# neuzxy/Distributed-TF-Serving

Measured on AMD Instinct MI355X. Metric: CTR scores/sec (whole node), higher is better.
Workload: dtype bf16; 1 GPU; model=deepfm (1Mx64 emb, 43 fields, MLP 1024-512-256), global_batch=16384, request_rows=512, parallelism=candidate-dp1 (one GPU, no fan-out), encoding=raw, aux_lane_cus=0

## Files before the change

### csrc/bindings_native.cpp

```cpp
#include <torch/extension.h>

#include <pybind11/stl.h>

#include <algorithm>
#include <cstring>

#include "runtime/batcher.h"
#include "runtime/arena.h"
#include "runtime/thread_pool.h"
#include "runtime/trace.h"
#include "wire/tensor_codec.h"
#include "live_bindings.h"
#include "runtime/narrow.h"
#include "net/hpack.h"
#include "runtime/numa.h"
#include "net/h2_client.h"

namespace py = pybind11;
using namespace dtfs;

namespace {

wire::DstType dst_type_of(const torch::Tensor& t) {
  switch (t.scalar_type()) {
    case torch::kInt32: return wire::DstType::I32;
    case torch::kInt64: return wire::DstType::I64;
    case torch::kFloat32: return wire::DstType::F32;
    case torch::kBFloat16: return wire::DstType::BF16;
    default: throw py::value_error("decode destination must be int32, int64, float32 or bfloat16");
  }
}

int wire_dtype_of(const torch::Tensor& t) {
  switch (t.scalar_type()) {
    case torch::kFloat32: return wire::DT_FLOAT;
    case torch::kFloat64: return wire::DT_DOUBLE;
    case torch::kInt32: return wire::DT_INT32;
    case torch::kInt64: return wire::DT_INT64;
    case torch::kBFloat16: return wire::DT_BFLOAT16;
    case torch::kFloat16: return wire::DT_HALF;
    default: throw py::value_error("unsupported tensor dtype for encoding");
  }
}

struct ParsedRequest {
  py::bytes holder;
  std::string storage;
  wire::PredictRequestView view;

  const wire::TensorView& get(const std::string& key) const {
    const wire::TensorView* t = view.find(key);
    if (!t) throw py::key_error("input '" + key + "' not found in PredictRequest");
    return *t;
  }
};

std::shared_ptr<ParsedRequest> parse_request(py::bytes data) {
// ... 192 lines not shown
      errs[k] = "input '" + b.ids_key + "': " + err;
      return;
    }
    if (wbase && b.wts_t[i]) {
      wire::DecodeOpts ow;
      ow.dst = wt;
      ow.cols = b.fields;
      ow.ld = wld;
      const bool ok = whole ? wire::decode_into(*b.wts_t[i], wbase + size_t(row * wld) * wes, n, ow, &err)
                            : wire::decode_into(sub(*b.wts_t[i], e0, e1), wbase + size_t(row * wld) * wes, n, ow, &err);
      if (!ok) errs[k] = "input '" + b.wts_key + "': " + err;
    }
  });
  for (size_t k = 0; k < items.size(); ++k)
    if (!errs[k].empty() && b.errors[items[k].req].empty()) b.errors[items[k].req] = errs[k];
}

using runtime::ArenaBatch;
using runtime::kArenaMaxRequests;
using runtime::kArenaPayloadOff;

void check_arena(const torch::Tensor& arena) {
  if (arena.device().type() != torch::kCPU || !arena.is_contiguous() || arena.scalar_type() != torch::kUInt8)
    throw py::value_error("arena must be a contiguous CPU uint8 tensor");
}

std::vector<std::pair<int64_t, int64_t>> arena_place(torch::Tensor arena, const std::vector<py::bytes>& reqs,
                                                     int64_t start) {
  check_arena(arena);
  std::vector<std::pair<const char*, size_t>> src(reqs.size());
  for (size_t i = 0; i < reqs.size(); ++i) {
    char* p;
    Py_ssize_t len;
    if (PyBytes_AsStringAndSize(reqs[i].ptr(), &p, &len) != 0) throw py::error_already_set();
    src[i] = {p, size_t(len)};
  }
  py::gil_scoped_release nogil;
  try {
    return runtime::arena_place(arena.data_ptr<uint8_t>(), arena.numel(), src, start);
  } catch (const std::invalid_argument& e) {
    py::gil_scoped_acquire g;
    throw py::value_error(e.what());
  }
}

ArenaBatch arena_build(torch::Tensor arena, const std::vector<std::pair<int64_t, int64_t>>& spans,
                       const std::string& ids_key, const std::string& wts_key, int64_t fields, int64_t max_rows,
                       int64_t varint_chunks, int64_t n_ranked) {
  check_arena(arena);
  py::gil_scoped_release nogil;
  try {
    return runtime::arena_build(arena.data_ptr<uint8_t>(), arena.numel(), spans, ids_key, wts_key, fields, max_rows,
                                varint_chunks, n_ranked);
  } catch (const std::invalid_argument& e) {
    py::gil_scoped_acquire g;
    throw py::value_error(e.what());
  }
}

void arena_unpack_cpu(torch::Tensor arena, torch::Tensor packed, int64_t fields) {
  check_arena(arena);
  if (packed.scalar_type() != torch::kInt64 || packed.dim() != 2 || !packed.is_contiguous())
    throw py::value_error("packed must be a contiguous int64 [B, W] tensor");
  if (packed.size(1) * 8 < 12 * fields) throw py::value_error("packed rows too narrow for the field count");
  const uint8_t* base = arena.data_ptr<uint8_t>();
  uint8_t* dst = reinterpret_cast<uint8_t*>(packed.data_ptr<int64_t>());
  const int64_t W = packed.size(1), B = packed.size(0);
  py::gil_scoped_release nogil;
  runtime::arena_unpack_cpu(base, dst, B, W, fields);
}

std::vector<py::bytes> encode_batch_responses(const std::string& name, const std::string& sig, py::object version,
                                              const std::string& key, torch::Tensor scores,
                                              const std::vector<int64_t>& rows, const std::vector<int64_t>& offsets,
                                              bool raw) {
  if (scores.device().type() != torch::kCPU || scores.scalar_type() != torch::kFloat32 || !scores.is_contiguous())
    throw py::value_error("scores must be a contiguous CPU fp32 tensor");
  if (rows.size() != offsets.size()) throw py::value_error("rows/offsets length mismatch");
  wire::ModelSpecOut spec;
  spec.name = name;
  spec.signature_name = sig;
  if (!version.is_none()) {
    spec.has_version = true;
    spec.version = version.cast<int64_t>();
  }
  const float* s = scores.data_ptr<float>();
  const int64_t ns = scores.numel();
  std::vector<std::string> outs(rows.size());
  {
    py::gil_scoped_release nogil;
    for (size_t i = 0; i < rows.size(); ++i) {
      if (offsets[i] < 0 || rows[i] < 0 || offsets[i] + rows[i] > ns) continue;
      wire::TensorOut t;
      t.key = key;
      t.dtype = wire::DT_FLOAT;
      t.shape = {rows[i]};
      t.data = s + offsets[i];
      t.n = rows[i];
      t.raw = raw;
      outs[i] = wire::encode_predict_response(spec, {t});
    }
  }
  std::vector<py::bytes> res;
  res.reserve(outs.size());
  for (auto& o : outs) res.emplace_back(o);
  return res;
// ... 268 lines not shown
      .def_property_readonly("output_filter", [](const ParsedRequest& r) { return r.view.output_filter; })
      .def("input_names", [](const ParsedRequest& r) {
        std::vector<std::string> k;
        for (const auto& kv : r.view.inputs) k.push_back(kv.first);
        return k;
      })
      .def("has_input", [](const ParsedRequest& r, const std::string& k) { return r.view.find(k) != nullptr; })
      .def("shape", [](const ParsedRequest& r, const std::string& k) { return r.get(k).shape; })
      .def("dtype", [](const ParsedRequest& r, const std::string& k) { return r.get(k).dtype; })
      .def("num_elements", [](const ParsedRequest& r, const std::string& k) { return r.get(k).num_elements(); })
      .def("num_values", [](const ParsedRequest& r, const std::string& k) {
        const auto& t = r.get(k);
        return t.content.n ? t.num_elements() : t.num_values;
      })
      .def("is_raw", [](const ParsedRequest& r, const std::string& k) { return r.get(k).content.n > 0; })
      .def("decode_into", &decode_into, py::arg("key"), py::arg("dst"), py::arg("offset") = 0,
           py::arg("id_modulo") = 0,
           "Decode input `key` (TF fill semantics) into dst[offset: offset+numel], narrowing dtypes.");

  m.def("parse_predict_request", &parse_request, py::arg("data"));

  py::class_<ParsedBatch, std::shared_ptr<ParsedBatch>>(m, "ParsedBatch")
      .def_readonly("rows", &ParsedBatch::rows)
      .def_readonly("offsets", &ParsedBatch::offsets)
      .def_readonly("errors", &ParsedBatch::errors)
      .def_readonly("total_rows", &ParsedBatch::total_rows)
      .def_readonly("fields", &ParsedBatch::fields)
      .def("__len__", [](const ParsedBatch& b) { return b.views.size(); })
      .def("model_name", [](const ParsedBatch& b, size_t i) { return b.views.at(i).model_name; })
      .def("signature_name", [](const ParsedBatch& b, size_t i) { return b.views.at(i).signature_name; })
      .def("version", [](const ParsedBatch& b, size_t i) -> py::object {
        const auto& v = b.views.at(i);
        return v.has_version ? py::object(py::int_(v.version)) : py::object(py::none());
      })
      .def("output_filter", [](const ParsedBatch& b, size_t i) { return b.views.at(i).output_filter; })
      .def("decode", &decode_batch_range, py::arg("ids_dst"), py::arg("wts_dst"), py::arg("begin") = 0,
           py::arg("end") = int64_t(1) << 62, py::arg("base_row") = 0, py::arg("id_modulo") = 0);

  py::class_<ArenaBatch>(m, "ArenaBatch")
      .def_readonly("rows", &ArenaBatch::rows)
      .def_readonly("offsets", &ArenaBatch::offsets)
      .def_readonly("errors", &ArenaBatch::errors)
      .def_readonly("total_rows", &ArenaBatch::total_rows)
      .def_readonly("used_bytes", &ArenaBatch::used_bytes)
      .def_readonly("n_valid", &ArenaBatch::n_valid)
      .def_readonly("n_decoded", &ArenaBatch::n_decoded)
      .def_readonly("n_gpu_varint", &ArenaBatch::n_gpu_varint);
  m.attr("ARENA_PAYLOAD_OFF") = kArenaPayloadOff;
  m.attr("ARENA_MAX_REQUESTS") = kArenaMaxRequests;
  m.def("arena_place", &arena_place, py::arg("arena"), py::arg("requests"), py::arg("start") = 0);
  m.def("arena_build", &arena_build, py::arg("arena"), py::arg("spans"), py::arg("ids_key") = "feat_ids",
        py::arg("wts_key") = "feat_wts", py::arg("fields") = 43, py::arg("max_rows") = int64_t(1) << 40,
        py::arg("varint_chunks") = 0, py::arg("n_ranked") = 0);
  m.def("arena_varint_capacity", &runtime::arena_varint_capacity, py::arg("max_rows"), py::arg("fields"),
        py::arg("max_requests") = runtime::kArenaMaxRequests);
  m.def("arena_unpack_cpu", &arena_unpack_cpu, py::arg("arena"), py::arg("packed"), py::arg("fields"));

  m.def("parse_batch", &parse_batch, py::arg("requests"), py::arg("ids_key") = "feat_ids",
        py::arg("wts_key") = "feat_wts", py::arg("fields") = 43,
        "Parse many serialized PredictRequests (GIL released); see ParsedBatch.decode.");
  m.def("encode_batch_responses", &encode_batch_responses, py::arg("model_name"), py::arg("signature_name"),
        py::arg("version"), py::arg("key"), py::arg("scores"), py::arg("rows"), py::arg("offsets"),
        py::arg("raw") = false);

  m.def(
      "encode_predict_response",
      [](const std::string& name, const std::string& sig, py::object version,
         const std::vector<std::pair<std::string, torch::Tensor>>& outputs, bool raw) {
        std::vector<torch::Tensor> keep;
        auto outs = tensors_out(outputs, raw, &keep);
        auto spec = spec_of(name, sig, version);
        std::string s;
        {
          py::gil_scoped_release nogil;
          s = wire::encode_predict_response(spec, outs);
        }
        return py::bytes(s);
      },
      py::arg("model_name"), py::arg("signature_name"), py::arg("version"), py::arg("outputs"),
      py::arg("raw") = false);

  m.def(
      "encode_predict_request",
      [](const std::string& name, const std::string& sig, py::object version,
         const std::vector<std::pair<std::string, torch::Tensor>>& inputs, bool raw,
         const std::vector<std::string>& output_filter) {
        std::vector<torch::Tensor> keep;
        auto ins = tensors_out(inputs, raw, &keep);
        auto spec = spec_of(name, sig, version);
        std::string s;
        {
          py::gil_scoped_release nogil;
          s = wire::encode_predict_request(spec, ins, output_filter);
        }
        return py::bytes(s);
      },
      py::arg("model_name"), py::arg("signature_name"), py::arg("version"), py::arg("inputs"),
      py::arg("raw") = false, py::arg("output_filter") = std::vector<std::string>{});

  m.def("f32_to_bf16_bits", [](float f) { return wire::f32_to_bf16(f); });

  py::class_<runtime::BatchItem>(m, "BatchItem")
      .def_readonly("ticket", &runtime::BatchItem::ticket)
      .def_readonly("rows", &runtime::BatchItem::rows)
      .def_readonly("enqueue_us", &runtime::BatchItem::enqueue_us)
      .def_readonly("deadline_us", &runtime::BatchItem::deadline_us);
// ... 86 lines not shown
```

### csrc/kernels/common.h

```cpp
#pragma once

#include <hip/hip_runtime.h>
#include <stdint.h>

namespace dtfs {
namespace kern {

typedef __bf16 bf16;
typedef __bf16 bf16x8 __attribute__((ext_vector_type(8)));
typedef __bf16 bf16x4 __attribute__((ext_vector_type(4)));
typedef float f32x4 __attribute__((ext_vector_type(4)));
typedef float f32x16 __attribute__((ext_vector_type(16)));
typedef int i32x4 __attribute__((ext_vector_type(4)));

constexpr int kWave = 64;

__device__ __forceinline__ float bf2f(bf16 x) { return float(x); }
__device__ __forceinline__ bf16 f2bf(float x) { return (bf16)x; }

__device__ __forceinline__ float wave_sum(float v) {
#pragma unroll
  for (int o = 32; o > 0; o >>= 1) v += __shfl_xor(v, o, 64);
  return v;
}
// ... 35 lines not shown
__device__ __forceinline__ uint32_t load_u32_unaligned(const uint8_t* p) {
  const uintptr_t a = reinterpret_cast<uintptr_t>(p);
  const uint32_t* w = reinterpret_cast<const uint32_t*>(a & ~uintptr_t(3));
  const int sh = int(a & 3);
  const uint32_t w0 = w[0];
  const uint32_t w1 = sh ? w[1] : 0u;
  return __builtin_amdgcn_alignbyte(w1, w0, sh);
}

constexpr int kArenaAllWeights = 1 << 30;
__device__ __forceinline__ int arena_narrow_wcols(const uint8_t* arena) {
  const int w = *reinterpret_cast<const int32_t*>(arena + 36);
  return w > 0 ? w : kArenaAllWeights;
}

__device__ __forceinline__ int arena_narrow_idb(const uint8_t* arena) {
  return *reinterpret_cast<const int32_t*>(arena + 40) == 3 ? 3 : 4;
}

constexpr uint32_t kWtsOffMask = 0x3fffffffu;
constexpr int kWtsF32 = 0, kWtsBf16 = 1, kWtsOnes = 2;

struct ArenaRow {
  const uint8_t* ids;
  const uint8_t* wts;
  bool narrow;
  int wcols;
  int idb;
  int wkind = kWtsF32;
};

__device__ __forceinline__ int64_t arena_narrow_id(const ArenaRow& ar, int f) {
  if (ar.idb == 3) return int64_t(load_u32_unaligned(ar.ids + 3 * f) & 0xffffffu);
  return int64_t(reinterpret_cast<const int32_t*>(ar.ids)[f]);
}

__device__ __forceinline__ float arena_narrow_w(const ArenaRow& ar, int f) {
  if (f >= ar.wcols) return 0.f;
  if (ar.wkind == kWtsOnes) return 1.f;
  if (ar.wkind == kWtsBf16) return __uint_as_float(uint32_t(reinterpret_cast<const uint16_t*>(ar.wts)[f]) << 16);
  return reinterpret_cast<const float*>(ar.wts)[f];
}

__device__ __forceinline__ ArenaRow arena_row_at(const uint8_t* payload, int2 o, int wcols, int idb) {
  ArenaRow r{payload + (o.x & 0x7fffffff), payload + (uint32_t(o.y) & kWtsOffMask), o.x < 0, kArenaAllWeights, 4};
  if (r.narrow) {
    r.wcols = wcols;
    r.idb = idb;
    r.wkind = int(uint32_t(o.y) >> 30);
  }
  return r;
}

__device__ __forceinline__ ArenaRow arena_row(const uint8_t* arena, int64_t payload_off, int64_t r) {
  const int64_t total = *reinterpret_cast<const int64_t*>(arena + 8);
  ArenaRow out{nullptr, nullptr, false, kArenaAllWeights, 4};
  if (r < total) {
    const uint8_t* payload = arena + payload_off;
    const int64_t rt = *reinterpret_cast<const int64_t*>(arena + 16);
    const int2 o = reinterpret_cast<const int2*>(payload + rt)[r];
    out = arena_row_at(payload, o, arena_narrow_wcols(arena), arena_narrow_idb(arena));
  }
  return out;
}

__device__ __forceinline__ void arena_feature(const ArenaRow& ar, int f, int64_t& id, float& w) {
  if (ar.narrow) {
    id = arena_narrow_id(ar, f);
    w = arena_narrow_w(ar, f);
  } else {
    id = int64_t(load_u64_unaligned(ar.ids + 8 * f));
    w = __uint_as_float(load_u32_unaligned(ar.wts + 4 * f));
  }
}

__device__ __forceinline__ int xcd_remap(int orig, int nwg) {
  constexpr int NX = 8;
  if (nwg <= NX) return orig;
  const int q = nwg / NX, r = nwg % NX;
  const int xcd = orig % NX, slot = orig / NX;
  const int base = xcd < r ? xcd * (q + 1) : r * (q + 1) + (xcd - r) * q;
  return base + slot;
}

}
}
```

### csrc/kernels/gather_mlp.hip

```cpp
#include <utility>

#include "asm_io.h"
#include "common.h"
#include "launchers.h"

namespace dtfs {
namespace kern {

typedef __bf16 bf16x2 __attribute__((ext_vector_type(2)));
typedef float f32x2 __attribute__((ext_vector_type(2)));

#ifdef DTFS_GM_STAMPS
__device__ unsigned long long g_gm_stamps[1024][4][16];
#define GM_T(k)                                             \
  do {                                                      \
    if (t == gm_t) gm_s[k] = __builtin_amdgcn_s_memtime(); \
  } while (0)
#define GM_AT(k)                              \
  do {                                        \
    gm_s[k] = __builtin_amdgcn_s_memtime(); \
  } while (0)
#else
#define GM_T(k) \
  do {          \
  } while (0)
#define GM_AT(k) \
  do {           \
  } while (0)
#endif

namespace {
template <int OFF>
__device__ __forceinline__ bf16x8 ds_read16_at(uint32_t addr) {
  bf16x8 v;
  asm volatile("ds_read_b128 %0, %1 offset:%2" : "=v"(v) : "v"(addr), "n"(OFF));
  return v;
}
template <int OFF>
__device__ __forceinline__ i32x4 ds_read16i_at(uint32_t addr) {
  i32x4 v;
  asm volatile("ds_read_b128 %0, %1 offset:%2" : "=v"(v) : "v"(addr), "n"(OFF));
  return v;
}
template <int OFF>
__device__ __forceinline__ int ds_read4_at(uint32_t addr) {
  int v;
  asm volatile("ds_read_b32 %0, %1 offset:%2" : "=v"(v) : "v"(addr), "n"(OFF));
  return v;
}
template <int OFF>
__device__ __forceinline__ void ds_write16_at(uint32_t addr, const i32x4& v) {
  asm volatile("ds_write_b128 %0, %1 offset:%2" ::"v"(addr), "v"(v), "n"(OFF) : "memory");
// ... 145 lines not shown
  const uint32_t sc_off = sc_r0 * 128 + ((sc_c ^ (sc_r0 & 7)) << 4);
  i32x4 sv[2];
  int swt[2];
  float fs[2][8], fsq[2] = {0.f, 0.f};
#pragma unroll
  for (int a = 0; a < 2; ++a)
#pragma unroll
    for (int d = 0; d < 8; ++d) fs[a][d] = 0.f;
  auto scale_read = [&](int u) {
    const uint32_t base = aring_lds + (u & (NS - 1)) * SLOT + sc_off;
    const uint32_t wb = wts_lds + min(u, F - 1) * (BM * 4) + 4 * sc_r0;
    sv[0] = ds_read16i_at<0>(base);
    swt[0] = ds_read4_at<0>(wb);
    sv[1] = ds_read16i_at<4096>(base);
    swt[1] = ds_read4_at<128>(wb);
  };
  auto scale_wait = [&] {
    asm volatile("s_waitcnt lgkmcnt(0)" : "+v"(sv[0]), "+v"(sv[1]), "+v"(swt[0]), "+v"(swt[1]));
  };
  i32x4 so[2];
  auto scale_pair = [&](int u, int q, int p) {
    const float wt = u < F ? __int_as_float(swt[q]) : 0.f;
    const float a = __uint_as_float(uint32_t(sv[q][p]) << 16) * wt;
    const float b = __uint_as_float(uint32_t(sv[q][p]) & 0xffff0000u) * wt;
    so[q][p] = __builtin_bit_cast(int, __builtin_convertvector((f32x2){a, b}, bf16x2));
    if constexpr (FM) {
      fs[q][2 * p] += a;
      fs[q][2 * p + 1] += b;
      fsq[q] += a * a;
      fsq[q] += b * b;
    }
    if (p == 3) ds_write16_at<0>(aring_lds + (u & (NS - 1)) * SLOT + sc_off + 4096 * q, so[q]);
  };

  f32x16 acc[8][2];
#pragma unroll
  for (int jn = 0; jn < 8; ++jn)
#pragma unroll
    for (int im = 0; im < 2; ++im)
#pragma unroll
      for (int g = 0; g < 16; ++g) acc[jn][im][g] = 0.f;
  auto mfma1 = [&](int jn, int im, int s) {
    acc[jn][im] = __builtin_amdgcn_mfma_f32_32x32x16_bf16(wf[jn][s], xf[im][s], acc[jn][im], 0, 0, 0);
  };
  auto pair = [&](int st, int k) {
    mfma1(2 * st + (k & 1), 0, k >> 1);
    mfma1(2 * st + (k & 1), 1, k >> 1);
  };
  auto fence = [] { __builtin_amdgcn_sched_barrier(0); };
  auto barrier = [] {
    __builtin_amdgcn_s_barrier();
    asm volatile("" ::: "memory");
  };
  auto wait_idx = [&] { asm volatile("s_waitcnt lgkmcnt(0)" : "+v"(aidx[0]), "+v"(aidx[1])::"memory"); };
#define WAIT_XS(N, s) wait_lgkm2<N>(xf[0][s], xf[1][s])

  auto vm_op = [&](int t, int g, int i) {
    if (g == 3) {
      load_w1(t, 6 + (i & 1), i >> 1);
    } else if (i < 8) {
      load_w1(t + 1, 2 * g + (i & 1), i >> 1);
    } else {
      stage_a(t + 3, g);
    }
  };

  reinterpret_cast<f32x4*>(b1s)[T] = reinterpret_cast<const f32x4*>(b1)[T];
  if (T < N2 / 4) reinterpret_cast<f32x4*>(b2s)[T] = reinterpret_cast<const f32x4*>(b2)[T];
  if (T < N3 / 4) {
    reinterpret_cast<f32x4*>(b3s)[T] = reinterpret_cast<const f32x4*>(b3)[T];
    reinterpret_cast<f32x4*>(hws)[T] = reinterpret_cast<const f32x4*>(hw)[T];
  }
#pragma unroll
  for (int g = 0; g < 3; ++g)
#pragma unroll
    for (int i = 0; i < 8; ++i) vm_op(-1, g, i);
  {
    constexpr int KR = FMAX / 4;
    const int rr = T & 63, f0 = T >> 6;
    const int b = m0 + rr;
    ArenaRow ar{nullptr, nullptr, false, kArenaAllWeights, 4};
    if (ea.arena && b < ea.B) ar = arena_row(static_cast<const uint8_t*>(ea.arena), kArenaPayloadOff, b);
    int64_t id[KR];
    float wv[KR];
#pragma unroll
    for (int k = 0; k < KR; ++k) {
      const int f = f0 + 4 * k;
      id[k] = 0;
      wv[k] = 0.f;
      if (f < F && b < ea.B) {
        if (ea.arena) {
          if (ar.ids) arena_feature(ar, f, id[k], wv[k]);
        } else {
          id[k] = ea.ids64 ? static_cast<const int64_t*>(ea.ids)[int64_t(b) * ea.ids_ld + f]
                           : int64_t(static_cast<const int32_t*>(ea.ids)[int64_t(b) * ea.ids_ld + f]);
          wv[k] = !ea.wts ? 1.f
                  : ea.wts16 ? __uint_as_float(uint32_t(static_cast<const uint16_t*>(ea.wts)[int64_t(b) * ea.wts_ld + f]) << 16)
                             : static_cast<const float*>(ea.wts)[int64_t(b) * ea.wts_ld + f];
        }
      }
    }
    float lsum = 0.f;
#pragma unroll
    for (int k = 0; k < KR; ++k) {
      const int f = f0 + 4 * k;
      if (f < F) {
        int64_t g = magic ? hash_row_magic(id[k], ea.modulo, magic) : hash_row(id[k], ea.modulo);
        g = g < 0 ? 0 : (g > Vm1 ? Vm1 : g);
        rows_l[f * BM + rr] = int32_t(g);
        wts_l[f * BM + rr] = wv[k];
        if (ea.lin) lsum += ea.lin[g] * wv[k];
      }
    }
    red[f0 * BM + rr] = lsum;
  }
  __syncthreads();
  if (T < BM) firstv[T] = ea.bias + red[T] + red[BM + T] + red[2 * BM + T] + red[3 * BM + T];
  read_idx(0);
  wait_idx();
  stage_a(0, 0);
  stage_a(0, 1);
  read_idx(1);
  wait_idx();
  stage_a(1, 0);
  stage_a(1, 1);
  read_idx(2);
  wait_idx();
  stage_a(2, 0);
  stage_a(2, 1);
  asm volatile("s_waitcnt vmcnt(2)" ::: "memory");
  barrier();
  scale_read(0);
  scale_wait();
#pragma unroll
  for (int q = 0; q < 2; ++q)
#pragma unroll
    for (int p = 0; p < 4; ++p) scale_pair(0, q, p);
  read_idx(3);
  wait_idx();
  barrier();
  read_xs(0, 0);
  read_xs(0, 1);
  read_xs(0, 2);
  GM_AT(1);

#pragma unroll 1
  for (int t = 0; t < F; ++t) {
    if constexpr (FM) {
      if (t == F - 1) {
#pragma unroll
        for (int a = 0; a < 2; ++a) {
          float part = -fsq[a];
#pragma unroll
          for (int d = 0; d < 8; ++d) part += fs[a][d] * fs[a][d];
          part += __shfl_xor(part, 1, 64);
          part += __shfl_xor(part, 2, 64);
          part += __shfl_xor(part, 4, 64);
          if (sc_c == 0) fmv[sc_r0 + 32 * a] = 0.5f * part;
        }
        __builtin_amdgcn_s_waitcnt(0xc07f);
      }
    }
    wait_vm8<18>(wf[0], wf[1]);
    GM_T(2);
    WAIT_XS(4, 0);
    pair(0, 0);
    vm_op(t, 3, 0);
    fence();
    pair(0, 1);
    vm_op(t, 3, 1);
    fence();
    read_xs(t, 3);
    WAIT_XS(4, 1);
    pair(0, 2);
    vm_op(t, 3, 2);
    fence();
    pair(0, 3);
    vm_op(t, 3, 3);
    fence();
    WAIT_XS(2, 2);
    pair(0, 4);
    vm_op(t, 3, 4);
    fence();
    pair(0, 5);
// ... 110 lines not shown
#pragma unroll
          for (int e = 0; e < 4; ++e) o[e] = f2bf(fmaxf(acc2[jn][im][4 * g4 + e] + b4[g4][e], lo2));
          *reinterpret_cast<bf16x4*>(smem + hswz(m, n >> 3, H2P) + 8 * he) = o;
        }
      }
    }
  }
  __syncthreads();
  GM_AT(11);

  {
    f32x16 acc3[2][2];
#pragma unroll
    for (int jn = 0; jn < 2; ++jn)
#pragma unroll
      for (int im = 0; im < 2; ++im)
#pragma unroll
        for (int g = 0; g < 16; ++g) acc3[jn][im][g] = 0.f;
    tail_gemm<2, N2 / 64, H2P>(W3p + int64_t(2 * w) * (N2 / 64) * 4 * 64, aring_lds, r32e, he, acc3);
    const float lo3 = act3 == 1 ? 0.f : -__builtin_huge_valf();
    float part[2] = {0.f, 0.f};
#pragma unroll
    for (int jn = 0; jn < 2; ++jn)
#pragma unroll
      for (int g4 = 0; g4 < 4; ++g4) {
        const int n = 64 * w + 32 * jn + 8 * g4 + 4 * he;
        const f32x4 bb = *reinterpret_cast<const f32x4*>(b3s + n);
        const f32x4 hh = *reinterpret_cast<const f32x4*>(hws + n);
#pragma unroll
        for (int im = 0; im < 2; ++im)
#pragma unroll
          for (int e = 0; e < 4; ++e) part[im] += fmaxf(acc3[jn][im][4 * g4 + e] + bb[e], lo3) * hh[e];
      }
#pragma unroll
    for (int im = 0; im < 2; ++im) {
      const float v = part[im] + __shfl_xor(part[im], 32, 64);
      if (he == 0) red[w * BM + 32 * im + r32e] = v;
    }
  }
  __syncthreads();
  if (tid_e < BM) {
    const int m = m0 + tid_e;
    if (m < M) {
      float s = hbias + firstv[tid_e];
      if constexpr (FM) s += fmv[tid_e];
#pragma unroll
      for (int ww = 0; ww < 4; ++ww) s += red[ww * BM + tid_e];
      y[m] = out_act == 2 ? sigmoidf(s) : s;
    }
  }
#ifdef DTFS_GM_STAMPS
  GM_AT(12);
  if (lane_e == 0 && blockIdx.x < 1024)
    for (int k = 0; k < 13; ++k) g_gm_stamps[blockIdx.x][w][k] = gm_s[k];
#endif
}

}

bool gather_mlp_ok(int64_t Mp, int N1, int K1, int N2, int N3, int F, int64_t V) {
  return N1 == 1024 && N2 == 512 && N3 == 256 && K1 == 64 * F && Mp % 64 == 0 && F >= 1 && F <= 64 && V >= 1 &&
         V <= (int64_t(1) << 25);
}

hipError_t launch_gather_mlp(const EmbedArgs& a, const void* W1p, const float* b1, const void* W2p, const float* b2,
                             int act2, const void* W3p, const float* b3, int act3, const float* hw, float hbias,
                             bool fm, int out_act, float* y, hipStream_t st) {
  if (a.B == 0) return hipSuccess;
  const int64_t Mp = (int64_t(a.B) + 63) / 64 * 64;
  if (!gather_mlp_ok(Mp, 1024, 64 * a.F, 512, 256, a.F, a.V) || a.B < 0 || a.modulo <= 0 || !a.table ||
      (!a.arena && !a.ids) || a.modulo_f || a.shard_lo_f || !W1p || !b1 || !W2p || !b2 || !W3p || !b3 || !hw || !y)
    return hipErrorInvalidValue;
  const uint64_t magic = a.modulo < (int64_t(1) << 32) ? ~uint64_t(0) / uint64_t(a.modulo) : 0;
  const int grid = int(Mp / 64);
  if (fm)
    hipLaunchKernelGGL((kern::gather_mlp_kernel<true>), dim3(grid), dim3(256), 0, st, a, magic, a.F,
                       static_cast<const kern::bf16x8*>(W1p), b1, static_cast<const kern::bf16x8*>(W2p), b2, act2,
                       static_cast<const kern::bf16x8*>(W3p), b3, act3, hw, hbias, a.B, out_act, y);
  else
    hipLaunchKernelGGL((kern::gather_mlp_kernel<false>), dim3(grid), dim3(256), 0, st, a, magic, a.F,
                       static_cast<const kern::bf16x8*>(W1p), b1, static_cast<const kern::bf16x8*>(W2p), b2, act2,
                       static_cast<const kern::bf16x8*>(W3p), b3, act3, hw, hbias, a.B, out_act, y);
  return hipGetLastError();
}

}
```

### distributed_tf_serving_amd/serving/arena.py

```python
from __future__ import annotations

from dataclasses import dataclass
from typing import List, Sequence, Tuple

import torch

from ..ops import native


@dataclass(frozen=True)
class ArenaLayout:
    fields: int
    max_rows: int
    max_requests: int = 1024
    gpu_varint: bool = True

    @property
    def varint_chunks(self) -> int:
        if not self.gpu_varint:
            return 0
        return native().arena_varint_capacity(self.max_rows, self.fields, self.max_requests)

    @property
    def varint_blocks(self) -> int:
        return min(1024, self.varint_chunks)

    def decode_varints(self, arena_dev: torch.Tensor) -> None:
        if self.gpu_varint:
            from ..ops import hip

            hip().arena_varint_decode(arena_dev, self.varint_blocks)

    @property
    def payload_off(self) -> int:
        return native().ARENA_PAYLOAD_OFF

    @property
    def capacity(self) -> int:
        per_row = 28 * self.fields + 8
        return (self.payload_off + self.max_rows * per_row + self.max_requests * 1024 + 128
                + 32 * self.varint_chunks)

    def alloc(self, device="cpu", pin: bool = False) -> torch.Tensor:
        return torch.zeros(self.capacity, dtype=torch.uint8, device=device, pin_memory=pin)

    def place(self, arena: torch.Tensor, requests: Sequence[bytes], start: int = 0) -> List[Tuple[int, int]]:
        return native().arena_place(arena, list(requests), start)

    def build(self, arena: torch.Tensor, spans: Sequence[Tuple[int, int]], ids_key="feat_ids", wts_key="feat_wts",
              n_ranked: int = 0):
        return native().arena_build(arena, list(spans), ids_key, wts_key, self.fields, self.max_rows,
                                    self.varint_chunks, int(n_ranked))

    def unpack_cpu(self, arena: torch.Tensor, packed: torch.Tensor) -> torch.Tensor:
        native().arena_unpack_cpu(arena, packed, self.fields)
        return packed
```

Before: 150.6 million scores/s.

## Stage contiguous arena tile runs into LDS with coalesced loads in gather_mlp

When all 64 rows of a tile are contiguous narrowed arena rows, the prologue loads the whole id and weight runs with 16-byte coalesced loads into spare LDS inside the h1 tile, then decodes per-feature ids and weights from LDS. This replaces scattered per-row unaligned global loads. It also overlaps the bias loads and the first A-staging with hashing, and adds a host-side mixed arena builder for pre-narrowed requests. The cost is extra LDS traffic and barriers, more register pressure, and a duplicated fallback path.

Result: faster. 155.6 million scores/s, median of 6 (+3.3%).

```diff
diff --git a/csrc/bindings_native.cpp b/csrc/bindings_native.cpp
--- a/csrc/bindings_native.cpp
+++ b/csrc/bindings_native.cpp
@@ -3,6 +3,7 @@
 #include <pybind11/stl.h>
 
 #include <algorithm>
+#include <climits>
 #include <cstring>
 
 #include "runtime/batcher.h"
@@ -301,6 +302,75 @@
   try {
     return runtime::arena_build(arena.data_ptr<uint8_t>(), arena.numel(), spans, ids_key, wts_key, fields, max_rows,
                                 varint_chunks, n_ranked);
+  } catch (const std::invalid_argument& e) {
+    py::gil_scoped_acquire g;
+    throw py::value_error(e.what());
+  }
+}
+
+ArenaBatch arena_build_mixed(torch::Tensor arena, const std::vector<py::object>& requests, int64_t modulo,
+                             int64_t id_bytes, int64_t narrow_wcols, int64_t wkind, const std::string& ids_key,
+                             const std::string& wts_key, int64_t fields, int64_t max_rows, int64_t varint_chunks,
+                             int64_t n_ranked) {
+  check_arena(arena);
+  if (id_bytes != 3 && id_bytes != 4) throw py::value_error("id_bytes must be 3 or 4");
+  if (modulo < 1 || modulo > (id_bytes == 3 ? int64_t(1) << 24 : int64_t(INT32_MAX)))
+    throw py::value_error("modulo does not fit the narrowed id width");
+  if (narrow_wcols < 0 || narrow_wcols > fields) throw py::value_error("narrow_wcols must be in [0, fields]");
+  if (wkind < -1 || wkind > runtime::kWtsOnes) throw py::value_error("wkind must be -1 (cheapest exact), 0, 1 or 2");
+  const int64_t wcols = narrow_wcols > 0 ? narrow_wcols : fields;
+  auto align64 = [](int64_t v) { return (v + 63) & ~int64_t(63); };
+  uint8_t* payload = arena.data_ptr<uint8_t>() + kArenaPayloadOff;
+  const int64_t cap = arena.numel() - kArenaPayloadOff;
+  std::vector<runtime::ArenaItem> items(requests.size());
+  std::vector<torch::Tensor> keep;
+  int64_t used = 0;
+  for (size_t i = 0; i < requests.size(); ++i) {
+    runtime::ArenaItem& it = items[i];
+    if (py::isinstance<py::bytes>(requests[i])) {
+      char* p;
+      Py_ssize_t len;
+      if (PyBytes_AsStringAndSize(requests[i].ptr(), &p, &len) != 0) throw py::error_already_set();
+      if (used + int64_t(len) > cap) throw py::value_error("arena too small for the batch");
+      it.off = used;
+      it.len = int64_t(len);
+      std::memcpy(payload + used, p, size_t(len));
+      used += (int64_t(len) + 7) & ~int64_t(7);
+      continue;
+    }
+    const auto pr = requests[i].cast<std::pair<torch::Tensor, torch::Tensor>>();
+    const torch::Tensor ids = pr.first.contiguous(), wts = pr.second.contiguous();
+    if (ids.device().type() != torch::kCPU || ids.scalar_type() != torch::kInt64 || ids.dim() != 2 ||
+        ids.size(1) != fields || wts.device().type() != torch::kCPU || wts.scalar_type() != torch::kFloat32 ||
+        wts.sizes() != ids.sizes())
+      throw py::value_error("a narrowed request is (ids int64 [n, fields], wts float32 [n, fields]) on the CPU");
+    keep.push_back(ids);
+    keep.push_back(wts);
+    const int64_t rows = ids.size(0), ne = rows * fields;
+    const uint8_t* wsrc = reinterpret_cast<const uint8_t*>(wts.data_ptr<float>());
+    const int exact = runtime::classify_weights(wsrc, rows, fields, wcols);
+    const bool holds = wkind < 0 || wkind == runtime::kWtsF32 || wkind == exact ||
+                       (wkind == runtime::kWtsBf16 && exact == runtime::kWtsOnes);
+    if (!holds) throw py::value_error("the forced weight form does not hold this request's weights exactly");
+    it.narrow = true;
+    it.rows = rows;
+    it.wkind = wkind < 0 ? exact : int(wkind);
+    it.ids_off = align64(used);
+    const int64_t ids_bytes = id_bytes == 3 ? 3 * ne + runtime::kNarrow24Slack : 4 * ne;
+    it.wts_off = align64(it.ids_off + ids_bytes);
+    used = it.wts_off + runtime::wts_bytes_per(it.wkind) * rows * wcols;
+    if (std::max(used, it.ids_off + ids_bytes) > cap) throw py::value_error("arena too small for the batch");
+    const uint8_t* isrc = reinterpret_cast<const uint8_t*>(ids.data_ptr<int64_t>());
+    if (id_bytes == 3)
+      runtime::narrow_ids24(isrc, payload + it.ids_off, ne, modulo);
+    else
+      runtime::narrow_ids(isrc, reinterpret_cast<int32_t*>(payload + it.ids_off), ne, modulo);
+    runtime::store_weights(wsrc, rows, fields, wcols, it.wkind, payload + it.wts_off);
+  }
+  py::gil_scoped_release nogil;
+  try {
+    return runtime::arena_build_items(arena.data_ptr<uint8_t>(), arena.numel(), items, ids_key, wts_key, fields,
+                                      max_rows, varint_chunks, narrow_wcols, id_bytes, n_ranked);
   } catch (const std::invalid_argument& e) {
     py::gil_scoped_acquire g;
     throw py::value_error(e.what());
@@ -675,6 +745,11 @@
   m.def("arena_build", &arena_build, py::arg("arena"), py::arg("spans"), py::arg("ids_key") = "feat_ids",
         py::arg("wts_key") = "feat_wts", py::arg("fields") = 43, py::arg("max_rows") = int64_t(1) << 40,
         py::arg("varint_chunks") = 0, py::arg("n_ranked") = 0);
+  m.def("arena_build_mixed", &arena_build_mixed, py::arg("arena"), py::arg("requests"), py::arg("modulo"),
+        py::arg("id_bytes") = 4, py::arg("narrow_wcols") = 0, py::arg("wkind") = -1, py::arg("ids_key") = "feat_ids",
+        py::arg("wts_key") = "feat_wts", py::arg("fields") = 43, py::arg("max_rows") = int64_t(1) << 40,
+        py::arg("varint_chunks") = 0, py::arg("n_ranked") = 0,
+        "Place serialized (bytes) and host-narrowed ((ids, wts) tensors) requests and build the arena.");
   m.def("arena_varint_capacity", &runtime::arena_varint_capacity, py::arg("max_rows"), py::arg("fields"),
         py::arg("max_requests") = runtime::kArenaMaxRequests);
   m.def("arena_unpack_cpu", &arena_unpack_cpu, py::arg("arena"), py::arg("packed"), py::arg("fields"));
diff --git a/csrc/kernels/common.h b/csrc/kernels/common.h
--- a/csrc/kernels/common.h
+++ b/csrc/kernels/common.h
@@ -111,16 +111,99 @@
   return r;
 }
 
+__device__ __forceinline__ bool arena_row_entry(const uint8_t* arena, int64_t payload_off, int64_t r, int2& o) {
+  const int64_t total = *reinterpret_cast<const int64_t*>(arena + 8);
+  if (r >= total) return false;
+  const int64_t rt = *reinterpret_cast<const int64_t*>(arena + 16);
+  o = reinterpret_cast<const int2*>(arena + payload_off + rt)[r];
+  return true;
+}
+
 __device__ __forceinline__ ArenaRow arena_row(const uint8_t* arena, int64_t payload_off, int64_t r) {
-  const int64_t total = *reinterpret_cast<const int64_t*>(arena + 8);
   ArenaRow out{nullptr, nullptr, false, kArenaAllWeights, 4};
-  if (r < total) {
-    const uint8_t* payload = arena + payload_off;
-    const int64_t rt = *reinterpret_cast<const int64_t*>(arena + 16);
-    const int2 o = reinterpret_cast<const int2*>(payload + rt)[r];
-    out = arena_row_at(payload, o, arena_narrow_wcols(arena), arena_narrow_idb(arena));
-  }
+  int2 o;
+  if (arena_row_entry(arena, payload_off, r, o))
+    out = arena_row_at(arena + payload_off, o, arena_narrow_wcols(arena), arena_narrow_idb(arena));
   return out;
+}
+
+struct ArenaTile {
+  bool ok;
+  uint32_t ids_off;
+  uint32_t wts_off;
+  int wts_stride;
+  int wkind;
+};
+
+__device__ __forceinline__ ArenaTile arena_tile_runs(int2 o, bool valid, int lane, int F, int wcols, int idb) {
+  const int x0 = __builtin_amdgcn_readfirstlane(o.x), y0 = __builtin_amdgcn_readfirstlane(o.y);
+  const int kind = int(uint32_t(y0) >> 30);
+  const int wb = kind == kWtsF32 ? 4 : kind == kWtsBf16 ? 2 : 0;
+  ArenaTile t{false, uint32_t(x0) & 0x7fffffffu, uint32_t(y0) & kWtsOffMask, wb * (wcols < F ? wcols : F), kind};
+  const bool row = valid && o.x < 0 && int(uint32_t(o.y) >> 30) == kind &&
+                   (uint32_t(o.x) & 0x7fffffffu) == t.ids_off + uint32_t(lane * idb * F) &&
+                   (uint32_t(o.y) & kWtsOffMask) == t.wts_off + uint32_t(lane * t.wts_stride);
+  const bool aligned = (idb == 3 || (t.ids_off & 3) == 0) && kind <= kWtsOnes &&
+                       (t.wts_off & (kind == kWtsF32 ? 3u : kind == kWtsBf16 ? 1u : 0u)) == 0;
+  t.ok = aligned && __builtin_amdgcn_ballot_w64(row) == ~uint64_t(0);
+  return t;
+}
+
+struct StagedRun {
+  i32x4 v[4];
+  int edge;
+  uint16_t half;
+  uint32_t nchunk, c0_lds;
+  int edge_lds, half_lds;
+};
+
+__device__ __forceinline__ uint32_t stage_phase(const uint8_t* p) { return uint32_t(reinterpret_cast<uintptr_t>(p) & 15); }
+
+template <bool HALF>
+__device__ __forceinline__ void stage_load(StagedRun& s, const uint8_t* p, uint32_t len, int T) {
+  const uintptr_t lo = reinterpret_cast<uintptr_t>(p), hi = lo + len, base = lo & ~uintptr_t(15);
+  const uintptr_t dlo = HALF ? (lo + 3) & ~uintptr_t(3) : lo & ~uintptr_t(3);
+  const uintptr_t dhi = HALF ? hi & ~uintptr_t(3) : (hi + 3) & ~uintptr_t(3);
+  uintptr_t c0 = (dlo + 15) & ~uintptr_t(15);
+  c0 = c0 < dhi ? c0 : dhi;
+  uintptr_t c1 = dhi & ~uintptr_t(15);
+  c1 = c1 > c0 ? c1 : c0;
+  s.nchunk = uint32_t((c1 - c0) >> 4);
+  s.c0_lds = uint32_t(c0 - base);
+#pragma unroll
+  for (int k = 0; k < 4; ++k) {
+    const uint32_t c = uint32_t(T) + 256u * k;
+    if (c < s.nchunk) s.v[k] = *reinterpret_cast<const i32x4*>(c0 + 16 * uintptr_t(c));
+  }
+  const int npre = int(c0 - dlo) >> 2, npost = int(dhi - c1) >> 2;
+  uintptr_t ea = 0;
+  if (T < npre) ea = dlo + 4 * uintptr_t(T);
+  if (T >= 4 && T - 4 < npost) ea = c1 + 4 * uintptr_t(T - 4);
+  s.edge_lds = -1;
+  if (ea) {
+    s.edge = *reinterpret_cast<const int*>(ea);
+    s.edge_lds = int(ea - base);
+  }
+  s.half_lds = -1;
+  if constexpr (HALF) {
+    uintptr_t ha = 0;
+    if (T == 8 && lo < dlo) ha = lo;
+    if (T == 9 && dhi < hi) ha = dhi;
+    if (ha) {
+      s.half = *reinterpret_cast<const uint16_t*>(ha);
+      s.half_lds = int(ha - base);
+    }
+  }
+}
+
+__device__ __forceinline__ void stage_store(const StagedRun& s, uint8_t* lds, int T) {
+#pragma unroll
+  for (int k = 0; k < 4; ++k) {
+    const uint32_t c = uint32_t(T) + 256u * k;
+    if (c < s.nchunk) *reinterpret_cast<i32x4*>(lds + s.c0_lds + 16 * c) = s.v[k];
+  }
+  if (s.edge_lds >= 0) *reinterpret_cast<int*>(lds + s.edge_lds) = s.edge;
+  if (s.half_lds >= 0) *reinterpret_cast<uint16_t*>(lds + s.half_lds) = s.half;
 }
 
 __device__ __forceinline__ void arena_feature(const ArenaRow& ar, int f, int64_t& id, float& w) {
diff --git a/csrc/kernels/gather_mlp.hip b/csrc/kernels/gather_mlp.hip
--- a/csrc/kernels/gather_mlp.hip
+++ b/csrc/kernels/gather_mlp.hip
@@ -1,3 +1,4 @@
+#include <type_traits>
 #include <utility>
 
 #include "asm_io.h"
@@ -249,6 +250,10 @@
     __builtin_amdgcn_s_barrier();
     asm volatile("" ::: "memory");
   };
+  auto lds_barrier = [&] {
+    asm volatile("s_waitcnt lgkmcnt(0)" ::: "memory");
+    barrier();
+  };
   auto wait_idx = [&] { asm volatile("s_waitcnt lgkmcnt(0)" : "+v"(aidx[0]), "+v"(aidx[1])::"memory"); };
 #define WAIT_XS(N, s) wait_lgkm2<N>(xf[0][s], xf[1][s])
 
@@ -262,71 +267,207 @@
     }
   };
 
-  reinterpret_cast<f32x4*>(b1s)[T] = reinterpret_cast<const f32x4*>(b1)[T];
-  if (T < N2 / 4) reinterpret_cast<f32x4*>(b2s)[T] = reinterpret_cast<const f32x4*>(b2)[T];
-  if (T < N3 / 4) {
-    reinterpret_cast<f32x4*>(b3s)[T] = reinterpret_cast<const f32x4*>(b3)[T];
-    reinterpret_cast<f32x4*>(hws)[T] = reinterpret_cast<const f32x4*>(hw)[T];
+  const uint8_t* const arena = static_cast<const uint8_t*>(ea.arena);
+  const int b = m0 + lane;
+  int wcols = kArenaAllWeights, idb = 4;
+  int2 ent = {0, 0};
+  bool have = false;
+  if (arena) {
+    const int64_t total = *reinterpret_cast<const int64_t*>(arena + 8);
+    const int64_t rt = *reinterpret_cast<const int64_t*>(arena + 16);
+    wcols = arena_narrow_wcols(arena);
+    idb = arena_narrow_idb(arena);
+    have = b < ea.B && b < total;
+    if (have) ent = reinterpret_cast<const int2*>(arena + kArenaPayloadOff + rt)[b];
   }
-#pragma unroll
-  for (int g = 0; g < 3; ++g)
-#pragma unroll
-    for (int i = 0; i < 8; ++i) vm_op(-1, g, i);
+  static_assert(N1 == 1024 && N2 == 512 && N3 == 256, "two 16-byte moves per thread");
+  const float* const bsrc = T < N2 / 4 ? b2 + 4 * T : T < (N2 + N3) / 4 ? b3 + (4 * T - N2) : hw + (4 * T - N2 - N3);
+  const f32x4 vb1 = reinterpret_cast<const f32x4*>(b1)[T];
+  const f32x4 vb2 = *reinterpret_cast<const f32x4*>(bsrc);
   {
     constexpr int KR = FMAX / 4;
-    const int rr = T & 63, f0 = T >> 6;
-    const int b = m0 + rr;
+    constexpr int STG_I = TWTS + FMAX * BM * 4, STG_W = STG_I + 16 * 1024 + 32;
+    static_assert(STG_W + 16 * 1024 + 32 <= HOFF, "the staged runs live inside the h1 tile, past the row tables");
+    const int rr = lane, f0 = T >> 6;
     ArenaRow ar{nullptr, nullptr, false, kArenaAllWeights, 4};
-    if (ea.arena && b < ea.B) ar = arena_row(static_cast<const uint8_t*>(ea.arena), kArenaPayloadOff, b);
-    int64_t id[KR];
-    float wv[KR];
-#pragma unroll
-    for (int k = 0; k < KR; ++k) {
-      const int f = f0 + 4 * k;
-      id[k] = 0;
-      wv[k] = 0.f;
-      if (f < F && b < ea.B) {
-        if (ea.arena) {
-          if (ar.ids) arena_feature(ar, f, id[k], wv[k]);
-        } else {
-          id[k] = ea.ids64 ? static_cast<const int64_t*>(ea.ids)[int64_t(b) * ea.ids_ld + f]
-                           : int64_t(static_cast<const int32_t*>(ea.ids)[int64_t(b) * ea.ids_ld + f]);
-          wv[k] = !ea.wts ? 1.f
-                  : ea.wts16 ? __uint_as_float(uint32_t(static_cast<const uint16_t*>(ea.wts)[int64_t(b) * ea.wts_ld + f]) << 16)
-                             : static_cast<const float*>(ea.wts)[int64_t(b) * ea.wts_ld + f];
+    ArenaTile tile{false, 0, 0, 0, 0};
+    if (arena) {
+      if (have) ar = arena_row_at(arena + kArenaPayloadOff, ent, wcols, idb);
+      tile = arena_tile_runs(ent, have, lane, F, wcols, idb);
+    }
+    const uint8_t* ip = nullptr;
+    const uint8_t* wp = nullptr;
+    if (tile.ok) {
+      ip = arena + kArenaPayloadOff + tile.ids_off;
+      wp = arena + kArenaPayloadOff + tile.wts_off;
+      StagedRun si, sw;
+      stage_load<false>(si, ip, uint32_t(BM * idb * F), T);
+      if (tile.wts_stride) stage_load<true>(sw, wp, uint32_t(BM * tile.wts_stride), T);
+      stage_store(si, smem + STG_I, T);
+      if (tile.wts_stride) stage_store(sw, smem + STG_W, T);
+    }
+#pragma unroll
+    for (int g = 0; g < 3; ++g)
+#pragma unroll
+      for (int i = 0; i < 8; ++i) vm_op(-1, g, i);
+    if (tile.ok) {
+      int64_t id[KR];
+      float wv[KR];
+      lds_barrier();
+      GM_AT(13);
+      const uint32_t irow = STG_I + stage_phase(ip) + uint32_t(rr * idb * F);
+      const uint32_t wrow = STG_W + stage_phase(wp) + uint32_t(rr * tile.wts_stride);
+      const int wb = tile.wkind == kWtsF32 ? 4 : tile.wkind == kWtsBf16 ? 2 : 0;
+      const uint32_t bfmask = tile.wkind == kWtsBf16 ? ~0u : 0u;
+      const uint32_t wmask = tile.wkind == kWtsOnes ? 0u : ~0u;
+      const uint32_t wone = tile.wkind == kWtsOnes ? 0x3f800000u : 0u;
+      const int nf = F < wcols ? F : wcols;
+      uint32_t d0[KR], d1[KR], dw[KR];
+#pragma unroll
+      for (int k = 0; k < KR; ++k) {
+        const int f = w + 4 * k;
+        if (f < F) {
+          const uint32_t* const d = reinterpret_cast<const uint32_t*>(smem + ((irow + idb * f) & ~3u));
+          d0[k] = d[0];
+          d1[k] = d[1];
+          dw[k] = *reinterpret_cast<const uint32_t*>(smem + ((wrow + wb * f) & ~3u));
         }
       }
-    }
-    float lsum = 0.f;
-#pragma unroll
-    for (int k = 0; k < KR; ++k) {
-      const int f = f0 + 4 * k;
-      if (f < F) {
-        int64_t g = magic ? hash_row_magic(id[k], ea.modulo, magic) : hash_row(id[k], ea.modulo);
-        g = g < 0 ? 0 : (g > Vm1 ? Vm1 : g);
-        rows_l[f * BM + rr] = int32_t(g);
-        wts_l[f * BM + rr] = wv[k];
-        if (ea.lin) lsum += ea.lin[g] * wv[k];
+      auto decode = [&](auto IDB3) {
+#pragma unroll
+        for (int k = 0; k < KR; ++k) {
+          const int f = w + 4 * k;
+          id[k] = 0;
+          wv[k] = 0.f;
+          if (f < F) {
+            const uint32_t v = __builtin_amdgcn_alignbyte(d1[k], d0[k], (irow + idb * f) & 3);
+            if constexpr (decltype(IDB3)::value) id[k] = int64_t(uint64_t(v & 0xffffffu));
+            else id[k] = int64_t(int32_t(v));
+            const uint32_t half = (wrow + wb * f) & 2 ? dw[k] & 0xffff0000u : dw[k] << 16;
+            const uint32_t bits = (((dw[k] & ~bfmask) | (half & bfmask)) & wmask) | wone;
+            wv[k] = __uint_as_float(f < nf ? bits : 0u);
+          }
+        }
+      };
+      auto finish = [&](auto IDB3, auto MAGIC) __attribute__((always_inline)) {
+        decode(IDB3);
+        int32_t g[KR];
+        float lv[KR];
+        auto resolve_k = [&](int k) {
+          const int f = w + 4 * k;
+          lv[k] = 0.f;
+          if (f < F) {
+            int64_t gg;
+            if constexpr (decltype(MAGIC)::value) gg = hash_row_magic(id[k], ea.modulo, magic);
+            else gg = hash_row(id[k], ea.modulo);
+            gg = gg < 0 ? 0 : (gg > Vm1 ? Vm1 : gg);
+            g[k] = int32_t(gg);
+            rows_l[f * BM + rr] = g[k];
+            wts_l[f * BM + rr] = wv[k];
+            if (ea.lin) lv[k] = ea.lin[g[k]];
+          }
+        };
+        resolve_k(0);
+        lds_barrier();
+        GM_AT(14);
+        read_idx(0);
+        wait_idx();
+        stage_a(0, 0);
+        stage_a(0, 1);
+        read_idx(1);
+        wait_idx();
+        stage_a(1, 0);
+        stage_a(1, 1);
+        read_idx(2);
+        wait_idx();
+        stage_a(2, 0);
+        stage_a(2, 1);
+#pragma unroll
+        for (int k = 1; k < KR; ++k) resolve_k(k);
+        float lsum = 0.f;
+#pragma unroll
+        for (int k = 0; k < KR; ++k)
+          if (w + 4 * k < F && ea.lin) lsum += lv[k] * wv[k];
+        red[w * BM + rr] = lsum;
+      };
+      if (magic) {
+        if (idb == 3) finish(std::true_type{}, std::true_type{});
+        else finish(std::false_type{}, std::true_type{});
+      } else {
+        if (idb == 3) finish(std::true_type{}, std::false_type{});
+        else finish(std::false_type{}, std::false_type{});
       }
-    }
-    red[f0 * BM + rr] = lsum;
+      asm volatile("s_waitcnt vmcnt(0)" ::: "memory");
+      reinterpret_cast<f32x4*>(b1s)[T] = vb1;
+      reinterpret_cast<f32x4*>(b2s)[T] = vb2;
+      __syncthreads();
+      GM_AT(15);
+      if (T < BM) firstv[T] = ea.bias + red[T] + red[BM + T] + red[2 * BM + T] + red[3 * BM + T];
+    } else {
+      int64_t id[KR];
+      float wv[KR];
+#pragma unroll
+      for (int k = 0; k < KR; ++k) {
+        const int f = f0 + 4 * k;
+        id[k] = 0;
+        wv[k] = 0.f;
+        if (f < F && b < ea.B) {
+          if (ea.arena) {
+            if (ar.ids) arena_feature(ar, f, id[k], wv[k]);
+          } else {
+            id[k] = ea.ids64 ? static_cast<const int64_t*>(ea.ids)[int64_t(b) * ea.ids_ld + f]
+                             : int64_t(static_cast<const int32_t*>(ea.ids)[int64_t(b) * ea.ids_ld + f]);
+            wv[k] = !ea.wts ? 1.f
+                    : ea.wts16 ? __uint_as_float(uint32_t(static_cast<const uint16_t*>(ea.wts)[int64_t(b) * ea.wts_ld + f]) << 16)
+                               : static_cast<const float*>(ea.wts)[int64_t(b) * ea.wts_ld + f];
+          }
+        }
+      }
+#ifdef DTFS_GM_STAMPS
+      asm volatile("s_waitcnt vmcnt(0)" : "+v"(id[0]), "+v"(wv[0])::"memory");
+      GM_AT(13);
+#endif
+      float lsum = 0.f;
+      auto hash_all = [&](auto MAGIC) __attribute__((always_inline)) {
+#pragma unroll
+        for (int k = 0; k < KR; ++k) {
+          const int f = f0 + 4 * k;
+          if (f < F) {
+            int64_t g;
+            if constexpr (decltype(MAGIC)::value) g = hash_row_magic(id[k], ea.modulo, magic);
+            else g = hash_row(id[k], ea.modulo);
+            g = g < 0 ? 0 : (g > Vm1 ? Vm1 : g);
+            rows_l[f * BM + rr] = int32_t(g);
+            wts_l[f * BM + rr] = wv[k];
+            if (ea.lin) lsum += ea.lin[g] * wv[k];
+          }
+        }
+      };
+      if (magic) hash_all(std::true_type{});
+      else hash_all(std::false_type{});
+      red[f0 * BM + rr] = lsum;
+      __syncthreads();
+      GM_AT(14);
+      reinterpret_cast<f32x4*>(b1s)[T] = vb1;
+      reinterpret_cast<f32x4*>(b2s)[T] = vb2;
+      if (T < BM) firstv[T] = ea.bias + red[T] + red[BM + T] + red[2 * BM + T] + red[3 * BM + T];
+      read_idx(0);
+      wait_idx();
+      stage_a(0, 0);
+      stage_a(0, 1);
+      read_idx(1);
+      wait_idx();
+      stage_a(1, 0);
+      stage_a(1, 1);
+      read_idx(2);
+      wait_idx();
+      stage_a(2, 0);
+      stage_a(2, 1);
+      asm volatile("s_waitcnt vmcnt(2)" ::: "memory");
+      barrier();
+      GM_AT(15);
+    }
   }
-  __syncthreads();
-  if (T < BM) firstv[T] = ea.bias + red[T] + red[BM + T] + red[2 * BM + T] + red[3 * BM + T];
-  read_idx(0);
-  wait_idx();
-  stage_a(0, 0);
-  stage_a(0, 1);
-  read_idx(1);
-  wait_idx();
-  stage_a(1, 0);
-  stage_a(1, 1);
-  read_idx(2);
-  wait_idx();
-  stage_a(2, 0);
-  stage_a(2, 1);
-  asm volatile("s_waitcnt vmcnt(2)" ::: "memory");
-  barrier();
   scale_read(0);
   scale_wait();
 #pragma unroll
@@ -543,7 +684,7 @@
 #ifdef DTFS_GM_STAMPS
   GM_AT(12);
   if (lane_e == 0 && blockIdx.x < 1024)
-    for (int k = 0; k < 13; ++k) g_gm_stamps[blockIdx.x][w][k] = gm_s[k];
+    for (int k = 0; k < 16; ++k) g_gm_stamps[blockIdx.x][w][k] = gm_s[k];
 #endif
 }
 
diff --git a/distributed_tf_serving_amd/serving/arena.py b/distributed_tf_serving_amd/serving/arena.py
--- a/distributed_tf_serving_amd/serving/arena.py
+++ b/distributed_tf_serving_amd/serving/arena.py
@@ -52,6 +52,12 @@
         return native().arena_build(arena, list(spans), ids_key, wts_key, self.fields, self.max_rows,
                                     self.varint_chunks, int(n_ranked))
 
+    def build_mixed(self, arena: torch.Tensor, requests: Sequence, modulo: int, id_bytes: int = 4,
+                    narrow_wcols: int = 0, wkind: int = -1, ids_key="feat_ids", wts_key="feat_wts", n_ranked: int = 0):
+        return native().arena_build_mixed(arena, list(requests), int(modulo), int(id_bytes), int(narrow_wcols),
+                                          int(wkind), ids_key, wts_key, self.fields, self.max_rows,
+                                          self.varint_chunks, int(n_ranked))
+
     def unpack_cpu(self, arena: torch.Tensor, packed: torch.Tensor) -> torch.Tensor:
         native().arena_unpack_cpu(arena, packed, self.fields)
         return packed
```
